# lucidrains/voicebox-pytorch

Hardware: AMD Instinct MI355X
Metric: mel-frames/sec train-step (fwd+bwd+allreduce+clip+Adam) (higher is better)
Workload: dtype f16/bf16 (fp16 forward operands, bf16 backward operands, fp32 accumulate/master); 1 GPU; VoiceBox dim 512 depth 12 heads 16 unconditional, 8x1024 frames per GPU, train; global_batch=8, seq_len=1024, parallelism=dp1

## Files before the change

voicebox-pytorch_amd/csrc/ops.hip:

```cpp
#include "common.hpp"
#include "reduce_roles.hpp"
#include <stdlib.h>

namespace {

VBX_DEV void unpack8_bf16(const uint4 p, float v[8]) {
  const unsigned w[4] = {p.x, p.y, p.z, p.w};
#pragma unroll
  for (int i = 0; i < 4; i++) {
    v[2 * i] = bf16_to_f32((u16)(w[i] & 0xffff));
    v[2 * i + 1] = bf16_to_f32((u16)(w[i] >> 16));
  }
}
VBX_DEV void unpack8_f16(const uint4 p, float v[8]) {
  const unsigned w[4] = {p.x, p.y, p.z, p.w};
#pragma unroll
  for (int i = 0; i < 4; i++) {
    v[2 * i] = f16_to_f32((u16)(w[i] & 0xffff));
    v[2 * i + 1] = f16_to_f32((u16)(w[i] >> 16));
  }
}
VBX_DEV uint4 pack8_h(const float v[8]) {
  return make_uint4(pack_f16x2_sat(v[0], v[1]), pack_f16x2_sat(v[2], v[3]), pack_f16x2_sat(v[4], v[5]), pack_f16x2_sat(v[6], v[7]));
}
// ... 111 lines not shown
  const int lane = threadIdx.x & 63;
  const long r = (long)blockIdx.x * 4 + (threadIdx.x >> 6);
  if (r >= rows) return;
  float s = 0.f;
  for (int d = lane * 4; d < D; d += 256) {
    const float4 a = *reinterpret_cast<const float4*>(x + r * D + d), b = *reinterpret_cast<const float4*>(w + d);
    s += a.x * b.x + a.y * b.y + a.z * b.z + a.w * b.w;
  }
  s = wave_sum(s);
  if (lane == 0) out[r] = s + (bias ? bias[0] : 0.f);
}
__global__ void cond_emb_bwd_kernel(const u16* __restrict__ demb, int ld, const long* __restrict__ ids, int T,
                                    const uint8_t* __restrict__ drop, long null_id, float* __restrict__ gtable, int B, int N, int E) {
  const long total = (long)B * N * E;
  for (long i = blockIdx.x * (long)blockDim.x + threadIdx.x; i < total; i += (long)gridDim.x * blockDim.x) {
    const long row = i / E;
    const int e = (int)(i - row * E);
    const int b = (int)(row / N), n = (int)(row - (long)b * N);
    const bool dropped = drop && drop[b];
    int i0, i1;
    float lam;
    interp_src(n, N, T, i0, i1, lam);
    const float g = bf16_to_f32(demb[row * ld + e]);
    const long id0 = dropped ? null_id : ids[(long)b * T + i0], id1 = dropped ? null_id : ids[(long)b * T + i1];
    if (T == N) {
      atomicAdd(gtable + id0 * E + e, g);
    } else {
      atomicAdd(gtable + id0 * E + e, (1.0f - lam) * g);
      atomicAdd(gtable + id1 * E + e, lam * g);
    }
  }
}

constexpr int CT = 64;
template <int MODE, int KS>
__global__ __launch_bounds__(256) void convpos_fwd_kernel(const float* __restrict__ e, const float* __restrict__ w,
                                                          const float* __restrict__ bias, const uint8_t* __restrict__ mask,
                                                          const float* __restrict__ dxs, float* __restrict__ out, int N,
                                                          int R, int D) {
  extern __shared__ float tile[];
  constexpr int ks = KS;
  const int half = ks / 2;
  const int n0 = blockIdx.x * CT, dbase = blockIdx.y * 64, b = blockIdx.z;
  const int dl = threadIdx.x & 63, ng = threadIdx.x >> 6;
  const int d = dbase + dl;
  const int rows = CT + ks - 1;
  for (int r = ng; r < rows; r += 4) {
    const int n = n0 + r - half;
    float v = 0.f;
    if (n >= 0 && n < N && d < D && (!mask || mask[(long)b * N + n])) v = e[((long)b * N + n) * D + d];
    tile[r * 64 + dl] = v;
  }
  __syncthreads();
  if (d >= D) return;
  float wr[KS];
#pragma unroll
  for (int k = 0; k < ks; k++) wr[k] = w[(long)d * ks + k];
  const float bb = bias[d];
  const int Np = N + R;
  for (int i = 0; i < 16; i++) {
    const int nl = ng * 16 + i, n = n0 + nl;
    if (n >= N) break;
    float acc = bb;
#pragma unroll
    for (int k = 0; k < ks; k++) acc += wr[k] * tile[(nl + k) * 64 + dl];
    const bool m = !mask || mask[(long)b * N + n];
    if (MODE == 0 || MODE == 2) {
      const float ev = e[((long)b * N + n) * D + d];
      out[((long)b * Np + R + n) * D + d] = ev + (m ? (MODE == 2 ? gelu_erf_libm(acc) : gelu_erf(acc)) : 0.f);
    } else {
      const float g = dxs[((long)b * Np + R + n) * D + d];
      out[((long)b * N + n) * D + d] = m ? g * gelu_erf_grad(acc) : 0.f;
    }
  }
}

__global__ void stack_rows_kernel(const float* __restrict__ src, float* __restrict__ dst, int B, int N, int R, int D, int to_stack) {
  const long total = (long)B * N * D / 4;
  const int D4 = D / 4;
  for (long i = blockIdx.x * (long)blockDim.x + threadIdx.x; i < total; i += (long)gridDim.x * blockDim.x) {
    const long row = i / D4;
    const int c = (int)(i - row * D4);
    const int b = (int)(row / N), n = (int)(row - (long)b * N);
    const long wide = ((long)b * (N + R) + R + n) * D4 + c, narrow = i;
    if (to_stack) reinterpret_cast<float4*>(dst)[wide] = reinterpret_cast<const float4*>(src)[narrow];
    else reinterpret_cast<float4*>(dst)[narrow] = reinterpret_cast<const float4*>(src)[wide];
  }
}

__global__ void unet_cat_kernel(const float* __restrict__ x, const float* __restrict__ skip, float scale, u16* __restrict__ o16,
                                u16* __restrict__ ob, long rows, int D) {
  const int cpr = D / 4;
  const long total = rows * 2 * cpr;
  for (long i = blockIdx.x * (long)blockDim.x + threadIdx.x; i < total; i += (long)gridDim.x * blockDim.x) {
    const long row = i / (2 * cpr);
    const int c = (int)(i - row * 2 * cpr);
    const bool second = c >= cpr;
    const int d = (second ? c - cpr : c) * 4;
    float4 v = *reinterpret_cast<const float4*>((second ? skip : x) + row * D + d);
    if (second) { v.x *= scale; v.y *= scale; v.z *= scale; v.w *= scale; }
    const long oo = row * 2 * D + (second ? D : 0) + d;
    if (o16) *reinterpret_cast<uint2*>(o16 + oo) = make_uint2(pack_f16x2_sat(v.x, v.y), pack_f16x2_sat(v.z, v.w));
    if (ob) *reinterpret_cast<uint2*>(ob + oo) = make_uint2(pack_bf16x2(v.x, v.y), pack_bf16x2(v.z, v.w));
  }
}
__global__ void unet_split_kernel(const float* __restrict__ dcat, float scale, float* __restrict__ dx, u16* __restrict__ dxb,
// ... 2 lines not shown
  const long total = rows * cpr;
  for (long i = blockIdx.x * (long)blockDim.x + threadIdx.x; i < total; i += (long)gridDim.x * blockDim.x) {
    const long row = i / cpr;
    const int d = (int)(i - row * cpr) * 4;
    const float4 a = *reinterpret_cast<const float4*>(dcat + row * 2 * D + d);
    float4 b = *reinterpret_cast<const float4*>(dcat + row * 2 * D + D + d);
    b.x *= scale; b.y *= scale; b.z *= scale; b.w *= scale;
    *reinterpret_cast<float4*>(dx + row * D + d) = a;
    if (dxb) *reinterpret_cast<uint2*>(dxb + row * D + d) = make_uint2(pack_bf16x2(a.x, a.y), pack_bf16x2(a.z, a.w));
    *reinterpret_cast<float4*>(dskip + row * D + d) = b;
  }
}
__global__ void unet_addskip_kernel(float* __restrict__ dx, u16* __restrict__ dxb, const float* __restrict__ dskip, long n4) {
  for (long i = blockIdx.x * (long)blockDim.x + threadIdx.x; i < n4; i += (long)gridDim.x * blockDim.x) {
    float4 a = reinterpret_cast<float4*>(dx)[i];
    const float4 b = reinterpret_cast<const float4*>(dskip)[i];
    a.x += b.x; a.y += b.y; a.z += b.z; a.w += b.w;
    reinterpret_cast<float4*>(dx)[i] = a;
    if (dxb) reinterpret_cast<uint2*>(dxb)[i] = make_uint2(pack_bf16x2(a.x, a.y), pack_bf16x2(a.z, a.w));
  }
}

__global__ void regs_fill_kernel(const float* __restrict__ reg, float* __restrict__ xs, int B, int Np, int R, int D) {
  const long total = (long)B * R * D;
  for (long i = blockIdx.x * (long)blockDim.x + threadIdx.x; i < total; i += (long)gridDim.x * blockDim.x) {
    const int b = (int)(i / ((long)R * D));
    const long rd = i - (long)b * R * D;
    xs[(long)b * Np * D + rd] = reg[rd];
  }
}

template <int KS>
__global__ __launch_bounds__(256) void convpos_bwd_kernel(const float* __restrict__ e, const float* __restrict__ w,
                                                          const uint8_t* __restrict__ mask, const float* __restrict__ dxs,
                                                          const float* __restrict__ dpre, float* __restrict__ de,
                                                          u16* __restrict__ deb, float* __restrict__ wpart, int N, int R,
                                                          int D) {
  extern __shared__ float sm[];
  constexpr int ks = KS;
  static_assert(KS <= 31, "wacc holds the taps in [0, KS) and the bias gradient in [31]");
  const int half = ks / 2;
  const int rows = CT + ks - 1;
  float* te = sm;
  float* tp = sm + rows * 64;
  const int n0 = blockIdx.x * CT, dbase = blockIdx.y * 64, b = blockIdx.z;
  const int dl = threadIdx.x & 63, ng = threadIdx.x >> 6;
  const int d = dbase + dl;
  for (int r = ng; r < rows; r += 4) {
    const int n = n0 + r - half;
    float ve = 0.f, vp = 0.f;
    if (n >= 0 && n < N && d < D) {
      if (!mask || mask[(long)b * N + n]) ve = e[((long)b * N + n) * D + d];
      vp = dpre[((long)b * N + n) * D + d];
    }
    te[r * 64 + dl] = ve;
    tp[r * 64 + dl] = vp;
  }
  __syncthreads();
  float wr[KS], wacc[32];
#pragma unroll
  for (int k = 0; k < 32; k++) wacc[k] = 0.f;
  if (d < D) {
#pragma unroll
    for (int k = 0; k < ks; k++) wr[k] = w[(long)d * ks + k];
    const int Np = N + R;
    for (int i = 0; i < 16; i++) {
      const int nl = ng * 16 + i, n = n0 + nl;
      if (n >= N) break;
      float acc = 0.f;
#pragma unroll
      for (int k = 0; k < ks; k++) acc += wr[k] * tp[(nl + 2 * half - k) * 64 + dl];
      const bool m = !mask || mask[(long)b * N + n];
      const float o = dxs[((long)b * Np + R + n) * D + d] + (m ? acc : 0.f);
      de[((long)b * N + n) * D + d] = o;
      if (deb) deb[((long)b * N + n) * D + d] = f32_to_bf16(o);
      const float dp = tp[(nl + half) * 64 + dl];
#pragma unroll
      for (int k = 0; k < ks; k++) wacc[k] += dp * te[(nl + k) * 64 + dl];
      wacc[31] += dp;
    }
  }
  __syncthreads();
  float* red = sm;
#pragma unroll
  for (int k = 0; k < 32; k++) red[(ng * 64 + dl) * 33 + k] = wacc[k];
  __syncthreads();
  const long chunk = (long)b * gridDim.x + blockIdx.x;
  for (int idx = threadIdx.x; idx < 64 * 32; idx += 256) {
    const int c = idx >> 5, k = idx & 31;
    if (dbase + c < D) {
      const float s = red[(0 * 64 + c) * 33 + k] + red[(1 * 64 + c) * 33 + k] + red[(2 * 64 + c) * 33 + k] +
                      red[(3 * 64 + c) * 33 + k];
      wpart[(chunk * D + dbase + c) * 64 + (k == 31 ? 63 : k)] = s;
    }
  }
}

__global__ void conv_wgrad_finalize_kernel(const float* __restrict__ wpart, int chunks, int D, int ks, float* __restrict__ dw,
                                           float* __restrict__ db) {
  const int idx = blockIdx.x * blockDim.x + threadIdx.x;
  if (idx >= D * 64) return;
  const int d = idx >> 6, k = idx & 63;
  if (k >= ks && k != 63) return;
  float s = 0.f;
  int c = 0;
  for (; c + 4 <= chunks; c += 4) {
    float v[4];
#pragma unroll
    for (int u = 0; u < 4; u++) v[u] = wpart[((long)(c + u) * D + d) * 64 + k];
#pragma unroll
    for (int u = 0; u < 4; u++) s += v[u];
  }
  for (; c < chunks; c++) s += wpart[((long)c * D + d) * 64 + k];
  if (k == 63) db[d] = s;
  else dw[(long)d * ks + k] = s;
}

__global__ void dreg_kernel(const float* __restrict__ dxs, float* __restrict__ dreg, int B, int Np, int R, int D) {
  const int i = blockIdx.x * blockDim.x + threadIdx.x;
  if (i >= R * D) return;
  float s = 0.f;
  for (int b = 0; b < B; b++) s += dxs[(long)b * Np * D + i];
  dreg[i] = s;
}

__global__ void time_four_kernel(const float* __restrict__ times, const float* __restrict__ wsin, float* __restrict__ four,
                                 int B, int D) {
  const int i = blockIdx.x * blockDim.x + threadIdx.x;
  if (i >= B * D) return;
  const int b = i / D, j = i - b * D, hd = D / 2;
  const int jj = j < hd ? j : j - hd;
  float f = times[b] * wsin[jj];
  f = f * 2.0f;
  f = f * 3.14159265358979323846f;
  four[i] = j < hd ? sinf(f) : cosf(f);
}
__global__ __launch_bounds__(256) void time_linear_kernel(const float* __restrict__ four, const float* __restrict__ w1,
                                                           const float* __restrict__ b1, float* __restrict__ pre,
                                                           float* __restrict__ temb, int B, int D, int Th) {
  const int lane = threadIdx.x & 63;
  const long o = (long)blockIdx.x * 4 + (threadIdx.x >> 6);
  if (o >= (long)B * Th) return;
  const int b = (int)(o / Th), i = (int)(o - (long)b * Th);
  float s = 0.f;
  for (int j = lane; j < D; j += 64) s += four[(long)b * D + j] * w1[(long)i * D + j];
  s = wave_sum(s);
  if (lane == 0) {
// ... 1118 lines not shown
  VBX_LAUNCH_CHECK();
  return 0;
}

extern "C" int vbx_rowdot(const float* x, const float* w, const float* bias, float* out, long rows, int D, void* stream) {
  VBX_REQUIRE(x && w && out && rows > 0 && D > 0 && D % 4 == 0, "vbx_rowdot: bad args");
  hipLaunchKernelGGL(rowdot_kernel, dim3((unsigned)cdiv(rows, 4L)), dim3(256), 0, ST, x, w, bias, out, rows, D);
  VBX_LAUNCH_CHECK();
  return 0;
}

extern "C" int vbx_cond_emb_bwd(const void* demb_bf16, int ld, const long* ids, int T, const uint8_t* drop_mask, long null_id,
                                float* gtable, int B, int N, int E, void* stream) {
  VBX_REQUIRE(demb_bf16 && ids && gtable && T > 0 && E > 0 && ld >= E, "vbx_cond_emb_bwd: bad args");
  hipLaunchKernelGGL(cond_emb_bwd_kernel, dim3(grid_for((long)B * N * E)), dim3(256), 0, ST, (const u16*)demb_bf16, ld, ids, T,
                     drop_mask, null_id, gtable, B, N, E);
  VBX_LAUNCH_CHECK();
  return 0;
}

#define VBX_CONV_KS_SWITCH(ks, CALL)                                                                                      \
  switch (ks) {                                                                                                           \
    case 1: CALL(1); break;   case 3: CALL(3); break;   case 5: CALL(5); break;   case 7: CALL(7); break;                 \
    case 9: CALL(9); break;   case 11: CALL(11); break; case 13: CALL(13); break; case 15: CALL(15); break;               \
    case 17: CALL(17); break; case 19: CALL(19); break; case 21: CALL(21); break; case 23: CALL(23); break;               \
    case 25: CALL(25); break; case 27: CALL(27); break; case 29: CALL(29); break; default: CALL(31); break;               \
  }
static inline bool conv_ks_ok(int ks) { return ks >= 1 && ks <= 31 && (ks & 1); }

static int convpos_fwd_impl(const float* e, const float* w, const float* bias, const uint8_t* mask, const float* reg, float* xs, int B,
                            int N, int R, int D, int ksize, bool libm, void* stream) {
  VBX_REQUIRE(e && w && bias && xs, "vbx_convpos_fwd: null pointer");
  VBX_REQUIRE(conv_ks_ok(ksize), "vbx_convpos_fwd: conv_pos_embed_kernel_size must be odd and <= 31 (got %d)", ksize);
  VBX_REQUIRE(R == 0 || reg, "vbx_convpos_fwd: register tokens missing");
  dim3 grid(cdiv(N, CT), cdiv(D, 64), B);
#define VBX_CALL(KS)                                                                                                           \
  if (libm)                                                                                                                    \
    hipLaunchKernelGGL((convpos_fwd_kernel<2, KS>), grid, dim3(256), (CT + KS - 1) * 64 * sizeof(float), ST, e, w, bias, mask, \
                       (const float*)nullptr, xs, N, R, D);                                                                    \
  else                                                                                                                         \
    hipLaunchKernelGGL((convpos_fwd_kernel<0, KS>), grid, dim3(256), (CT + KS - 1) * 64 * sizeof(float), ST, e, w, bias, mask, \
                       (const float*)nullptr, xs, N, R, D)
  VBX_CONV_KS_SWITCH(ksize, VBX_CALL)
#undef VBX_CALL
  VBX_LAUNCH_CHECK();
  if (R > 0) {
    hipLaunchKernelGGL(regs_fill_kernel, dim3(grid_for((long)B * R * D)), dim3(256), 0, ST, reg, xs, B, N + R, R, D);
    VBX_LAUNCH_CHECK();
  }
  return 0;
}

extern "C" int vbx_convpos_fwd(const float* e, const float* w, const float* bias, const uint8_t* mask, const float* reg,
                               float* xs, int B, int N, int R, int D, int ksize, void* stream) {
  return convpos_fwd_impl(e, w, bias, mask, reg, xs, B, N, R, D, ksize, false, stream);
}
extern "C" int vbx_convpos_fwd_libm(const float* e, const float* w, const float* bias, const uint8_t* mask, const float* reg,
                                    float* xs, int B, int N, int R, int D, int ksize, void* stream) {
  return convpos_fwd_impl(e, w, bias, mask, reg, xs, B, N, R, D, ksize, true, stream);
}

extern "C" int vbx_stack_input(const float* x, const float* reg, float* xs, int B, int N, int R, int D, void* stream) {
  VBX_REQUIRE(x && xs && B > 0 && N > 0 && R >= 0 && D % 4 == 0 && (R == 0 || reg), "vbx_stack_input: bad args");
  hipLaunchKernelGGL(stack_rows_kernel, dim3(grid_for((long)B * N * D / 4)), dim3(256), 0, ST, x, xs, B, N, R, D, 1);
  VBX_LAUNCH_CHECK();
  if (R > 0) {
    hipLaunchKernelGGL(regs_fill_kernel, dim3(grid_for((long)B * R * D)), dim3(256), 0, ST, reg, xs, B, N + R, R, D);
    VBX_LAUNCH_CHECK();
  }
  return 0;
}

extern "C" int vbx_unet_cat(const float* x, const float* skip, float scale, void* cat_f16, void* cat_bf16, long rows, int D, void* stream) {
  VBX_REQUIRE(x && skip && (cat_f16 || cat_bf16) && rows > 0 && D > 0 && D % 4 == 0, "vbx_unet_cat: bad args");
  hipLaunchKernelGGL(unet_cat_kernel, dim3(grid_for(rows * D / 2)), dim3(256), 0, ST, x, skip, scale, (u16*)cat_f16, (u16*)cat_bf16, rows, D);
  VBX_LAUNCH_CHECK();
  return 0;
}
extern "C" int vbx_unet_split(const float* dcat, float scale, float* dx, void* dx_bf16, float* dskip, long rows, int D, void* stream) {
  VBX_REQUIRE(dcat && dx && dskip && rows > 0 && D > 0 && D % 4 == 0, "vbx_unet_split: bad args");
  hipLaunchKernelGGL(unet_split_kernel, dim3(grid_for(rows * D / 4)), dim3(256), 0, ST, dcat, scale, dx, (u16*)dx_bf16, dskip, rows, D);
  VBX_LAUNCH_CHECK();
  return 0;
}
extern "C" int vbx_unet_addskip(float* dx, void* dx_bf16, const float* dskip, long n, void* stream) {
  VBX_REQUIRE(dx && dskip && n > 0 && n % 4 == 0, "vbx_unet_addskip: bad args");
  hipLaunchKernelGGL(unet_addskip_kernel, dim3(grid_for(n / 4)), dim3(256), 0, ST, dx, (u16*)dx_bf16, dskip, n / 4);
  VBX_LAUNCH_CHECK();
  return 0;
}

extern "C" int vbx_stack_input_bwd(const float* dxs, float* dx, float* dreg, int B, int N, int R, int D, void* stream) {
  VBX_REQUIRE(dxs && dx && B > 0 && N > 0 && R >= 0 && D % 4 == 0, "vbx_stack_input_bwd: bad args");
  hipLaunchKernelGGL(stack_rows_kernel, dim3(grid_for((long)B * N * D / 4)), dim3(256), 0, ST, dxs, dx, B, N, R, D, 0);
  VBX_LAUNCH_CHECK();
  if (R > 0 && dreg) {
    hipLaunchKernelGGL(dreg_kernel, dim3(cdiv((long)R * D, 256)), dim3(256), 0, ST, dxs, dreg, B, N + R, R, D);
    VBX_LAUNCH_CHECK();
  }
  return 0;
}

extern "C" int vbx_convpos_bwd_chunks(int B, int N) { return B * cdiv(N, CT); }

extern "C" int vbx_convpos_bwd(const float* e, const float* w, const float* bias, const uint8_t* mask, const float* dxs,
                               float* dpre_tmp, float* de, void* de_bf16, float* wpart, float* dreg, int B, int N, int R,
                               int D, int ksize, void* stream) {
  VBX_REQUIRE(e && w && bias && dxs && dpre_tmp && de && wpart, "vbx_convpos_bwd: null pointer");
  VBX_REQUIRE(conv_ks_ok(ksize), "vbx_convpos_bwd: conv_pos_embed_kernel_size must be odd and <= 31 (got %d)", ksize);
  dim3 grid(cdiv(N, CT), cdiv(D, 64), B);
  const int rows = CT + ksize - 1;
#define VBX_CALL(KS)                                                                                                            \
  hipLaunchKernelGGL((convpos_fwd_kernel<1, KS>), grid, dim3(256), rows * 64 * sizeof(float), ST, e, w, bias, mask, dxs, dpre_tmp, \
                     N, R, D)
  VBX_CONV_KS_SWITCH(ksize, VBX_CALL)
#undef VBX_CALL
  VBX_LAUNCH_CHECK();
  size_t lds = (size_t)(2 * rows * 64) * sizeof(float);
  if (lds < (size_t)4 * 64 * 33 * sizeof(float)) lds = (size_t)4 * 64 * 33 * sizeof(float);
  static bool attr[32] = {};
#define VBX_CALL(KS)                                                                                                              \
  {                                                                                                                               \
    if (!attr[KS]) {                                                                                                              \
      (void)hipFuncSetAttribute(reinterpret_cast<const void*>(convpos_bwd_kernel<KS>), hipFuncAttributeMaxDynamicSharedMemorySize, \
                                (int)lds);                                                                                        \
      attr[KS] = true;                                                                                                            \
    }                                                                                                                             \
    hipLaunchKernelGGL(convpos_bwd_kernel<KS>, grid, dim3(256), lds, ST, e, w, mask, dxs, dpre_tmp, de, (u16*)de_bf16, wpart, N,   \
                       R, D);                                                                                                     \
  }
  VBX_CONV_KS_SWITCH(ksize, VBX_CALL)
#undef VBX_CALL
  VBX_LAUNCH_CHECK();
  if (R > 0 && dreg) {
    hipLaunchKernelGGL(dreg_kernel, dim3(cdiv((long)R * D, 256)), dim3(256), 0, ST, dxs, dreg, B, N + R, R, D);
    VBX_LAUNCH_CHECK();
  }
  return 0;
}

extern "C" int vbx_conv_wgrad_finalize(const float* wpart, int chunks, int D, int ksize, float* dw, float* db, void* stream) {
  VBX_REQUIRE(wpart && dw && db && ksize < 63, "vbx_conv_wgrad_finalize: bad args");
  hipLaunchKernelGGL(conv_wgrad_finalize_kernel, dim3(cdiv((long)D * 64, 256)), dim3(256), 0, ST, wpart, chunks, D, ksize, dw, db);
  VBX_LAUNCH_CHECK();
  return 0;
}

extern "C" int vbx_time_embed_fwd(const float* times, const float* w_sin, const float* w1, const float* b1, float* four,
                                  float* pre, float* temb, int B, int D, int Th, void* stream) {
  VBX_REQUIRE(times && w_sin && w1 && b1 && four && pre && temb && D % 2 == 0, "vbx_time_embed_fwd: bad args");
  hipLaunchKernelGGL(time_four_kernel, dim3(cdiv((long)B * D, 256)), dim3(256), 0, ST, times, w_sin, four, B, D);
  VBX_LAUNCH_CHECK();
  hipLaunchKernelGGL(time_linear_kernel, dim3(cdiv((long)B * Th, 4)), dim3(256), 0, ST, four, w1, b1, pre, temb, B, D, Th);
  VBX_LAUNCH_CHECK();
  return 0;
}

extern "C" int vbx_time_embed_bwd_scratch_floats(int B, int D) { return (1 + TB_SLICES) * B * D; }

extern "C" int vbx_time_embed_bwd(const float* times, const float* w_sin, const float* w1, const float* four,
                                  const float* pre, const float* dtemb, float* dw_sin, float* dw1, float* db1,
                                  float* scratch, int B, int D, int Th, void* stream) {
  VBX_REQUIRE(times && w_sin && w1 && four && pre && dtemb && dw_sin && dw1 && db1 && scratch, "vbx_time_embed_bwd: null");
  hipLaunchKernelGGL(time_bwd_w1_kernel, dim3(cdiv((long)Th * D, 256)), dim3(256), 0, ST, four, pre, dtemb, dw1, db1, B, D, Th);
  VBX_LAUNCH_CHECK();
  hipLaunchKernelGGL(time_bwd_four_kernel, dim3(cdiv(D, 64), B, TB_SLICES), dim3(64), 0, ST, w1, pre, dtemb, scratch + (long)B * D,
                     B, D, Th);
  VBX_LAUNCH_CHECK();
  hipLaunchKernelGGL(sum_rows_kernel, dim3(cdiv((long)B * D, 64)), dim3(256), 0, ST, scratch + (long)B * D, (long)TB_SLICES,
                     (long)B * D, scratch, (long)B * D, 0);
  VBX_LAUNCH_CHECK();
  hipLaunchKernelGGL(time_bwd_wsin_kernel, dim3(cdiv(D / 2, 256)), dim3(256), 0, ST, times, four, scratch, dw_sin, B, D);
  VBX_LAUNCH_CHECK();
  return 0;
}

// ... 434 lines not shown
```

voicebox-pytorch_amd/csrc/runtime.hip:

```cpp
#include "common.hpp"
#include <stdlib.h>
#include <algorithm>
#include <string.h>
#include <string>
#include <vector>

namespace {

inline size_t al256(size_t x) { return (x + 255) & ~(size_t)255; }

struct Carver {
  char* base;
  size_t off = 0;
  explicit Carver(void* b) : base((char*)b) {}
  template <class T>
  T* take(size_t n) {
    off = al256(off);
    T* p = base ? (T*)(base + off) : nullptr;
    off += n * sizeof(T);
    return p;
  }
};

struct Dims {
// ... 44 lines not shown
    w.layer[l].w1 = c.take<u16>((size_t)2 * d.Fp * d.D);
    w.layer[l].w1h = c.take<u16>((size_t)2 * d.Fp * d.D);
    w.layer[l].b1 = c.take<float>(2 * d.Fp);
    w.layer[l].w2 = c.take<u16>((size_t)d.D * d.Fp);
    w.layer[l].w2h = c.take<u16>((size_t)d.D * d.Fp);
    w.layer[l].glw = m->gateloop ? c.take<u16>((size_t)3 * d.D * d.D) : nullptr;
    w.layer[l].glwh = m->gateloop ? c.take<u16>((size_t)3 * d.D * d.D) : nullptr;
    if (m->unet && l >= d.L / 2) {
      w.layer[l].skw = c.take<u16>((size_t)2 * d.D * d.D);
      w.layer[l].skwh = c.take<u16>((size_t)2 * d.D * d.D);
    }
  }
  w.bytes = al256(c.off);
}

struct ALayer {
  u16 *hn1, *hn1h, *q16, *k16, *qb, *kb, *v, *vh, *o, *oh, *hn2, *hn2h, *h1, *g, *gh;
  float *qrn, *krn, *lse;
  unsigned *dbr = nullptr, *dbc = nullptr;
  u16 *hg = nullptr, *hgh = nullptr;
  float *glp = nullptr, *glh = nullptr, *gls = nullptr;
};
struct Acts {
  u16 *embed_in, *embed_inh;
  u16 *xcb = nullptr, *dxc = nullptr;
  float *e, *four, *pre, *temb, *ada;
  std::vector<float*> xs;
  std::vector<float*> xc, dskip;
  u16 *cat16 = nullptr, *catb = nullptr;
  float* dcat = nullptr;
  std::vector<ALayer> layer;
  u16 *hf, *hfh;
  float *pred, *per_b;
  float *dx, *dq, *dk, *delta, *slabs, *npart, *npart2, *cpart, *dada, *dtemb, *cs_scratch, *cs_layers, *gpart, *tmp2d, *ada_scratch, *dpre, *de, *wpart,
      *tscratch;
  u16 *dxb, *dg, *dh1, *dhn, *dO, *dqkv, *deb, *dpb, *gl_dp, *demb;
  char* attn_scratch = nullptr;
  u16* dxb2 = nullptr;
  float* gl_ds;
  size_t slab_floats;
  size_t np_stride = 0, cp_stride = 0, cs_stride = 0, gp_stride = 0;
  size_t bytes;
};

int wgrad_splits(long I, long J, long K) {
  const long tiles = ((I + 127) / 128) * ((J + 127) / 128);
  const long smax = (K + 511) / 512;
  int best = 1;
  double best_cost = 1e30;
  for (int s = 1; s <= 16 && s <= smax; s++) {
    const long W = tiles * s;
    const long n = (W + 255) / 256;
    const double eff = n >= 3 ? 1.0 : (n == 2 ? 0.85 : 0.6);
    const double ksteps = (double)((K + s - 1) / s) / 32.0;
    const double gemm = (double)n * ksteps * 0.27 / eff;
    const double slab = (double)s * (double)I * (double)J * 8.0 / 4.0e6;
    const double cost = gemm + slab;
    if (cost < best_cost) { best_cost = cost; best = s; }
  }
  return best;
}

bool group_wgrad() { return vbx_gemm_path() != 1; }
struct WgradGroup {
  vbx_gemm_desc d[4];
  int n = 0;
};
// ... 93 lines not shown
    auto upd = [&](long I, long J, long K) {
      const int s1 = wgrad_splits(I, J, K);
      const size_t n = (size_t)(s1 > s3 ? s1 : s3) * I * J;
      if (n > sf) sf = n;
    };
    upd(3 * d.I, d.D, d.M); upd(d.D, d.I, d.M); upd(2 * d.Fp, d.D, d.M); upd(d.D, d.Fp, d.M);
    upd(d.D, d.Ke, d.M0); upd(d.Dop, d.D, d.M0);
    if (d.Lc) upd(d.D, d.Kp, 2 * d.M0);
    if (m->gateloop) upd(3 * d.D, d.D, d.M);
    if (m->unet) upd(d.D, 2 * d.D, d.M);
    a.slab_floats = sf;
    a.slabs = c.take<float>(4 * sf);
    const size_t nreg = (m->gateloop || m->unet) ? 1 : (size_t)d.L;
    a.np_stride = (size_t)d.B * vbx_rmsnorm_bwd_chunks(d.Np) * 2 * d.D;
    a.cp_stride = (size_t)d.B * vbx_rmsnorm_bwd_chunks(d.Np) * d.D;
    a.npart = c.take<float>(a.np_stride * nreg);
    a.npart2 = c.take<float>(a.np_stride * nreg);
    a.cpart = c.take<float>(a.cp_stride * nreg);
    a.dada = c.take<float>((size_t)d.B * d.J);
    a.dtemb = c.take<float>((size_t)d.B * d.Th);
    size_t cs = (size_t)vbx_colsum_scratch_floats((int)d.M, 2 * d.Fp);
    if (cs < (size_t)vbx_geglu_bwd_colsum_slabs() * 2 * d.Fp) cs = (size_t)vbx_geglu_bwd_colsum_slabs() * 2 * d.Fp;
    a.cs_scratch = c.take<float>(cs);
    a.cs_stride = (size_t)vbx_geglu_bwd_colsum_slabs() * 2 * d.Fp;
    a.cs_layers = c.take<float>(a.cs_stride * nreg);
    {
      const int r1 = vbx_qknorm_rope_bwd_gpart_rows(d.B), r2 = d.B * vbx_attn_bwd_fused_tiles(d.Np);
      a.gp_stride = (size_t)2 * (r1 > r2 ? r1 : r2) * d.H * 64;
      a.gpart = c.take<float>(a.gp_stride * nreg);
    }
    a.tmp2d = c.take<float>(2 * d.D);
    a.ada_scratch = c.take<float>(std::max((size_t)vbx_adaln_proj_bwd_scratch_floats(d.B, d.Th, 4 * d.D),
                                           (size_t)vbx_adaln_dtemb_all_scratch_floats(d.L, d.B, d.Th, 4 * d.D)));
    a.dpre = c.take<float>((size_t)d.M0 * d.D);
    a.de = c.take<float>((size_t)d.M0 * d.D);
    a.deb = c.take<u16>((size_t)d.M0 * d.D);
    a.dpb = c.take<u16>((size_t)d.M0 * d.Dop);
    a.wpart = c.take<float>((size_t)vbx_convpos_bwd_chunks(d.B, d.N) * d.D * 64);
    a.tscratch = c.take<float>((size_t)vbx_time_embed_bwd_scratch_floats(d.B, d.D));
    a.gl_ds = m->gateloop ? c.take<float>((size_t)d.M * d.D) : nullptr;
    a.gl_dp = m->gateloop ? c.take<u16>((size_t)d.M * 3 * d.D) : nullptr;
    a.demb = d.E ? c.take<u16>((size_t)d.M0 * d.E) : nullptr;
    if (d.Lc) {
      a.xcb = c.take<u16>((size_t)2 * d.M0 * d.Kp);
      a.dxc = c.take<u16>((size_t)2 * d.M0 * d.D);
    }
    a.dxb2 = c.take<u16>((size_t)d.M * d.D);
    a.attn_scratch = c.take<char>(vbx_attn_bwd_scratch_bytes(d.B, d.H, d.Np));
    if (m->unet) {
      a.catb = c.take<u16>((size_t)d.M * 2 * d.D);
      a.dcat = c.take<float>((size_t)d.M * 2 * d.D);
      for (int p = 0; p < d.L / 2; p++) a.dskip[p] = c.take<float>((size_t)d.M * d.D);
    }
  }
  a.bytes = al256(c.off);
}

struct ProfRec {
  const char* label;
  hipEvent_t e0, e1;
};
struct Prof {
  bool on = false;
  std::vector<ProfRec> recs;
};
Prof g_prof;
struct ProfScope {
// ... 521 lines not shown
    if (l == 0) {
      ProfScope ps("adaLN dtemb (all)", st);
      CK(vbx_adaln_dtemb_all(w.adah, a.dada, a.dtemb, a.ada_scratch, d.L, d.B, d.Th, 4 * d.D, stream));
    }
    return 0;
  }
  return vbx_adaln_proj_bwd(m->stack_only ? io->cond : a.temb, w.adah + (size_t)l * 4 * d.D * d.Th, dada_l,
                            m->adaln_factors ? nullptr : Gd + o[VBX_L_G1W], Gd + o[VBX_L_G1B], a.dtemb,
                            a.ada_scratch, d.B, d.Th, 4 * d.D, l == d.L - 1 ? 0 : 1, stream);
}

extern "C" int vbx_model_backward_embed(const vbx_model* m, const vbx_io* io, void* stream) {
  CK(check_model(m));
  VBX_REQUIRE(m->training && m->grads && io && (m->stack_only ? io->dx != nullptr : io->times != nullptr),
              "vbx_model_backward_embed: needs a training forward");
  hipStream_t st = (hipStream_t)stream;
  const Dims d = dims_of(m);
  WPack w;
  carve_wpack(m, w);
  Acts a;
  carve_acts(m, a);
  const float* P = m->params;
  float* Gd = m->grads;
  const long* G = m->off;
  if (m->stack_only) {
    CK(vbx_stack_input_bwd(a.dx, io->dx, d.R ? Gd + G[VBX_P_REG] : nullptr, d.B, d.N, d.R, d.D, stream));
    if (!m->plain_norm && io->dcond &&
        hipMemcpyAsync(io->dcond, a.dtemb, (size_t)d.B * d.Th * sizeof(float), hipMemcpyDeviceToDevice, st) != hipSuccess) {
      vbx_set_error("vbx_model_backward_embed: copy of d(cond) failed");
      return VBX_EINVAL;
    }
    return 0;
  }
  CK(vbx_convpos_bwd(a.e, P + G[VBX_P_CONVW], P + G[VBX_P_CONVB], io->attn_mask, a.dx, a.dpre, a.de, a.deb, a.wpart,
                     d.R ? Gd + G[VBX_P_REG] : nullptr, d.B, d.N, d.R, d.D, d.ks, stream));
  CK(vbx_conv_wgrad_finalize(a.wpart, vbx_convpos_bwd_chunks(d.B, d.N), d.D, d.ks, Gd + G[VBX_P_CONVW], Gd + G[VBX_P_CONVB], stream));
  CK(wgrad(a.deb, d.D, a.embed_in, d.Ke, d.D, d.Ke, d.M0, a.slabs, Gd + G[VBX_P_EMBW], d.D, d.Ke, 0, 0, st));
  if (d.E) {
    WPack w;
    carve_wpack(m, w);
    CK(gemm_nn_bf16(a.deb, d.D, w.embb + d.Din, d.Ke, (int)d.M0, d.E, d.D, a.demb, d.E, st));
    if (hipMemsetAsync(Gd + G[VBX_P_CEMB], 0, (size_t)m->V1 * d.E * sizeof(float), st) != hipSuccess) {
      vbx_set_error("vbx_model_backward_embed: memset of the embedding gradient failed");
      return VBX_EINVAL;
    }
    CK(vbx_cond_emb_bwd(a.demb, d.E, io->cond_ids, io->T, io->drop_mask, io->null_id, Gd + G[VBX_P_CEMB], d.B, d.N, d.E, stream));
  }
  if (d.Lc) {
    WPack w;
    carve_wpack(m, w);
    CK(gemm_nn_bf16(a.deb, d.D, w.embb, d.Ke, (int)d.M0, d.D, d.D, a.dxc, d.D, st));
    CK(gemm_nn_bf16(a.deb, d.D, w.embb + d.D + d.E, d.Ke, (int)d.M0, d.D, d.D, a.dxc + (size_t)d.M0 * d.D, d.D, st));
    vbx_gemm_desc g{};
    g.mode = VBX_GEMM_TN; g.epilogue = VBX_EPI_SPLITK; g.M = d.D; g.N = d.Kp; g.K = (int)(2 * d.M0); g.lda = d.D; g.ldb = d.Kp;
    g.A = a.dxc; g.B = a.xcb; g.C = a.slabs; g.splits = wgrad_splits(d.D, d.Kp, 2 * d.M0);
    CK(vbx_gemm(&g, st));
    CK(vbx_proj_in_wgrad_reduce(a.slabs, g.splits, d.D, d.Lc, Gd + G[VBX_P_PINW], Gd + G[VBX_P_PINB], stream));
  }
  CK(vbx_colsum_f32(a.de, (int)d.M0, d.D, d.D, Gd + G[VBX_P_EMBB], a.cs_scratch, stream));
  CK(vbx_time_embed_bwd(io->times, P + G[VBX_P_SINW], P + G[VBX_P_T1W], a.four, a.pre, a.dtemb, Gd + G[VBX_P_SINW],
                        Gd + G[VBX_P_T1W], Gd + G[VBX_P_T1B], a.tscratch, d.B, d.D, d.Th, stream));
  return 0;
}

extern "C" int vbx_model_adam_segments(const vbx_model* m, long n_flat, vbx_adam_seg* out, int max_segs, long* total_blocks) {
  CK(check_model(m));
  VBX_REQUIRE(n_flat > 0 && total_blocks, "vbx_model_adam_segments: bad args");
// ... 118 lines not shown
```

Baseline: 961,300 mel-frames/s.

## Fuse conv-pos backward pre-activation recompute into one kernel with register-tiled frames

The backward pass for the positional depthwise conv now recomputes the pre-activation inside the main backward kernel, using a halo tile of the input. This removes the separate MODE-1 forward launch and the fp32 dpre buffer round-trip through global memory. Both forward and backward are re-tiled: each thread owns two channels and eight frames, with float4 tile fills and float2 LDS accesses, and weight-grad partials are pre-reduced with warp shuffles into a 32-wide wpart layout. The cost is redundant conv compute over the halo rows, more registers per thread, and a new requirement that D be a multiple of 4.

After: 970,100 mel-frames/s (median of 6 runs). Within noise of the previous version (+0.9%).

```diff
diff --git a/voicebox-pytorch_amd/csrc/ops.hip b/voicebox-pytorch_amd/csrc/ops.hip
--- a/voicebox-pytorch_amd/csrc/ops.hip
+++ b/voicebox-pytorch_amd/csrc/ops.hip
@@ -167,46 +167,85 @@
   }
 }
 
-constexpr int CT = 64;
-template <int MODE, int KS>
+constexpr int CV_RUN = 128, CV_CW = 32, CV_FR = 8, CV_P = 36;
+
+template <int ROWS>
+__device__ __forceinline__ void conv_fill_tile(float* __restrict__ tile, const float* __restrict__ src, const uint8_t* __restrict__ mrow,
+                                               int nfirst, int N, int D, int dbase) {
+  constexpr int IT = (ROWS * 8 + 255) / 256;
+  float4 v[IT];
+  bool ok[IT];
+#pragma unroll
+  for (int it = 0; it < IT; it++) {
+    const int idx = threadIdx.x + it * 256, r = idx >> 3, c4 = idx & 7;
+    const int n = nfirst + r, d = dbase + c4 * 4;
+    const int nc = min(max(n, 0), N - 1), dc = min(d, D - 4);
+    ok[it] = n >= 0 && n < N && d < D && (!mrow || mrow[nc]);
+    v[it] = *reinterpret_cast<const float4*>(src + (long)nc * D + dc);
+  }
+#pragma unroll
+  for (int it = 0; it < IT; it++) {
+    const int idx = threadIdx.x + it * 256, r = idx >> 3, c4 = idx & 7;
+    if (idx < ROWS * 8) *reinterpret_cast<float4*>(tile + r * CV_P + c4 * 4) = ok[it] ? v[it] : make_float4(0.f, 0.f, 0.f, 0.f);
+  }
+}
+
+template <int LIBM, int KS>
 __global__ __launch_bounds__(256) void convpos_fwd_kernel(const float* __restrict__ e, const float* __restrict__ w,
                                                           const float* __restrict__ bias, const uint8_t* __restrict__ mask,
-                                                          const float* __restrict__ dxs, float* __restrict__ out, int N,
-                                                          int R, int D) {
+                                                          float* __restrict__ out, int N, int R, int D) {
   extern __shared__ float tile[];
-  constexpr int ks = KS;
-  const int half = ks / 2;
-  const int n0 = blockIdx.x * CT, dbase = blockIdx.y * 64, b = blockIdx.z;
-  const int dl = threadIdx.x & 63, ng = threadIdx.x >> 6;
-  const int d = dbase + dl;
-  const int rows = CT + ks - 1;
-  for (int r = ng; r < rows; r += 4) {
-    const int n = n0 + r - half;
-    float v = 0.f;
-    if (n >= 0 && n < N && d < D && (!mask || mask[(long)b * N + n])) v = e[((long)b * N + n) * D + d];
-    tile[r * 64 + dl] = v;
-  }
+  constexpr int half = KS / 2, rows = CV_RUN + KS - 1;
+  const int n0 = blockIdx.x * CV_RUN, dbase = blockIdx.y * CV_CW, b = blockIdx.z;
+  const int q = threadIdx.x & 15, f0 = (threadIdx.x >> 4) * CV_FR;
+  const int d = dbase + 2 * q;
+  const uint8_t* mrow = mask ? mask + (long)b * N : nullptr;
+  const float* eb = e + (long)b * N * D;
+  float wr[2][KS], acc[CV_FR][2];
+  if (d < D) {
+#pragma unroll
+    for (int k = 0; k < KS; k++) {
+      wr[0][k] = w[(long)d * KS + k];
+      wr[1][k] = w[(long)(d + 1) * KS + k];
+    }
+#pragma unroll
+    for (int i = 0; i < CV_FR; i++) {
+      acc[i][0] = bias[d];
+      acc[i][1] = bias[d + 1];
+    }
+  }
+  conv_fill_tile<rows>(tile, eb, mrow, n0 - half, N, D, dbase);
   __syncthreads();
   if (d >= D) return;
-  float wr[KS];
-#pragma unroll
-  for (int k = 0; k < ks; k++) wr[k] = w[(long)d * ks + k];
-  const float bb = bias[d];
+#pragma unroll
+  for (int j = 0; j < CV_FR + KS - 1; j++) {
+    const float2 x = *reinterpret_cast<const float2*>(tile + (f0 + j) * CV_P + 2 * q);
+#pragma unroll
+    for (int i = 0; i < CV_FR; i++) {
+      const int k = j - i;
+      if (k >= 0 && k < KS) {
+        acc[i][0] += wr[0][k] * x.x;
+        acc[i][1] += wr[1][k] * x.y;
+      }
+    }
+  }
   const int Np = N + R;
-  for (int i = 0; i < 16; i++) {
-    const int nl = ng * 16 + i, n = n0 + nl;
+#pragma unroll
+  for (int i = 0; i < CV_FR; i++) {
+    const int n = n0 + f0 + i;
     if (n >= N) break;
-    float acc = bb;
-#pragma unroll
-    for (int k = 0; k < ks; k++) acc += wr[k] * tile[(nl + k) * 64 + dl];
-    const bool m = !mask || mask[(long)b * N + n];
-    if (MODE == 0 || MODE == 2) {
-      const float ev = e[((long)b * N + n) * D + d];
-      out[((long)b * Np + R + n) * D + d] = ev + (m ? (MODE == 2 ? gelu_erf_libm(acc) : gelu_erf(acc)) : 0.f);
+    const bool m = !mrow || mrow[n];
+    float2 o;
+    if (m) {
+      const float2 ev = *reinterpret_cast<const float2*>(tile + (f0 + i + half) * CV_P + 2 * q);
+      o.x = ev.x + (LIBM ? gelu_erf_libm(acc[i][0]) : gelu_erf(acc[i][0]));
+      o.y = ev.y + (LIBM ? gelu_erf_libm(acc[i][1]) : gelu_erf(acc[i][1]));
     } else {
-      const float g = dxs[((long)b * Np + R + n) * D + d];
-      out[((long)b * N + n) * D + d] = m ? g * gelu_erf_grad(acc) : 0.f;
-    }
+      const float2 ev = *reinterpret_cast<const float2*>(eb + (long)n * D + d);
+      o.x = ev.x + 0.f;
+      o.y = ev.y + 0.f;
+    }
+    *reinterpret_cast<float2*>(out + ((long)b * Np + R + n) * D + d) = o;
   }
 }
 
@@ -275,66 +314,144 @@
 
 template <int KS>
 __global__ __launch_bounds__(256) void convpos_bwd_kernel(const float* __restrict__ e, const float* __restrict__ w,
-                                                          const uint8_t* __restrict__ mask, const float* __restrict__ dxs,
-                                                          const float* __restrict__ dpre, float* __restrict__ de,
+                                                          const float* __restrict__ bias, const uint8_t* __restrict__ mask,
+                                                          const float* __restrict__ dxs, float* __restrict__ de,
                                                           u16* __restrict__ deb, float* __restrict__ wpart, int N, int R,
                                                           int D) {
   extern __shared__ float sm[];
-  constexpr int ks = KS;
-  static_assert(KS <= 31, "wacc holds the taps in [0, KS) and the bias gradient in [31]");
-  const int half = ks / 2;
-  const int rows = CT + ks - 1;
+  constexpr int half = KS / 2;
+  constexpr int RE = CV_RUN + 4 * half, RP = CV_RUN + 2 * half;
+  constexpr int PB = (RP + 15) / 16;
   float* te = sm;
-  float* tp = sm + rows * 64;
-  const int n0 = blockIdx.x * CT, dbase = blockIdx.y * 64, b = blockIdx.z;
-  const int dl = threadIdx.x & 63, ng = threadIdx.x >> 6;
-  const int d = dbase + dl;
-  for (int r = ng; r < rows; r += 4) {
-    const int n = n0 + r - half;
-    float ve = 0.f, vp = 0.f;
-    if (n >= 0 && n < N && d < D) {
-      if (!mask || mask[(long)b * N + n]) ve = e[((long)b * N + n) * D + d];
-      vp = dpre[((long)b * N + n) * D + d];
-    }
-    te[r * 64 + dl] = ve;
-    tp[r * 64 + dl] = vp;
-  }
+  float* tp = sm + RE * CV_P;
+  const int n0 = blockIdx.x * CV_RUN, dbase = blockIdx.y * CV_CW, b = blockIdx.z;
+  const int q = threadIdx.x & 15, g = threadIdx.x >> 4;
+  const int d = dbase + 2 * q;
+  const bool active = d < D;
+  const int Np = N + R;
+  const uint8_t* mrow = mask ? mask + (long)b * N : nullptr;
+  const float* dxb = dxs + ((long)b * Np + R) * D;
+  float wr[2][KS];
+  float bb[2] = {0.f, 0.f};
+  if (active) {
+#pragma unroll
+    for (int k = 0; k < KS; k++) {
+      wr[0][k] = w[(long)d * KS + k];
+      wr[1][k] = w[(long)(d + 1) * KS + k];
+    }
+    bb[0] = bias[d];
+    bb[1] = bias[d + 1];
+  }
+  conv_fill_tile<RE>(te, e + (long)b * N * D, mrow, n0 - 2 * half, N, D, dbase);
+  conv_fill_tile<RP>(tp, dxb, mrow, n0 - half, N, D, dbase);
   __syncthreads();
-  float wr[KS], wacc[32];
-#pragma unroll
-  for (int k = 0; k < 32; k++) wacc[k] = 0.f;
-  if (d < D) {
-#pragma unroll
-    for (int k = 0; k < ks; k++) wr[k] = w[(long)d * ks + k];
-    const int Np = N + R;
-    for (int i = 0; i < 16; i++) {
-      const int nl = ng * 16 + i, n = n0 + nl;
+  if (active) {
+    const int rb = g * PB;
+    float acc[PB][2];
+#pragma unroll
+    for (int i = 0; i < PB; i++) {
+      acc[i][0] = bb[0];
+      acc[i][1] = bb[1];
+    }
+#pragma unroll
+    for (int j = 0; j < PB + KS - 1; j++) {
+      const float2 x = *reinterpret_cast<const float2*>(te + min(rb + j, RE - 1) * CV_P + 2 * q);
+#pragma unroll
+      for (int i = 0; i < PB; i++) {
+        const int k = j - i;
+        if (k >= 0 && k < KS) {
+          acc[i][0] += wr[0][k] * x.x;
+          acc[i][1] += wr[1][k] * x.y;
+        }
+      }
+    }
+#pragma unroll
+    for (int i = 0; i < PB; i++) {
+      const int r = rb + i;
+      if (r < RP) {
+        float2* pp = reinterpret_cast<float2*>(tp + r * CV_P + 2 * q);
+        const float2 gv = *pp;
+        *pp = make_float2(gv.x * gelu_erf_grad(acc[i][0]), gv.y * gelu_erf_grad(acc[i][1]));
+      }
+    }
+  }
+  __syncthreads();
+  float wacc[2][32];
+#pragma unroll
+  for (int k = 0; k < 32; k++) wacc[0][k] = wacc[1][k] = 0.f;
+  if (active) {
+    const int f0 = g * CV_FR;
+    float acc[CV_FR][2];
+#pragma unroll
+    for (int i = 0; i < CV_FR; i++) acc[i][0] = acc[i][1] = 0.f;
+#pragma unroll
+    for (int j = CV_FR + 2 * half - 1; j >= 0; j--) {
+      const float2 x = *reinterpret_cast<const float2*>(tp + (f0 + j) * CV_P + 2 * q);
+#pragma unroll
+      for (int i = 0; i < CV_FR; i++) {
+        const int k = i + 2 * half - j;
+        if (k >= 0 && k < KS) {
+          acc[i][0] += wr[0][k] * x.x;
+          acc[i][1] += wr[1][k] * x.y;
+        }
+      }
+    }
+    float2 dp[CV_FR];
+#pragma unroll
+    for (int i = 0; i < CV_FR; i++) {
+      dp[i] = *reinterpret_cast<const float2*>(tp + (f0 + i + half) * CV_P + 2 * q);
+      wacc[0][31] += dp[i].x;
+      wacc[1][31] += dp[i].y;
+    }
+#pragma unroll
+    for (int j = 0; j < CV_FR + KS - 1; j++) {
+      const float2 x = *reinterpret_cast<const float2*>(te + (f0 + half + j) * CV_P + 2 * q);
+#pragma unroll
+      for (int i = 0; i < CV_FR; i++) {
+        const int k = j - i;
+        if (k >= 0 && k < KS) {
+          wacc[0][k] += dp[i].x * x.x;
+          wacc[1][k] += dp[i].y * x.y;
+        }
+      }
+    }
+#pragma unroll
+    for (int i = 0; i < CV_FR; i++) {
+      const int n = n0 + f0 + i;
       if (n >= N) break;
-      float acc = 0.f;
-#pragma unroll
-      for (int k = 0; k < ks; k++) acc += wr[k] * tp[(nl + 2 * half - k) * 64 + dl];
-      const bool m = !mask || mask[(long)b * N + n];
-      const float o = dxs[((long)b * Np + R + n) * D + d] + (m ? acc : 0.f);
-      de[((long)b * N + n) * D + d] = o;
-      if (deb) deb[((long)b * N + n) * D + d] = f32_to_bf16(o);
-      const float dp = tp[(nl + half) * 64 + dl];
-#pragma unroll
-      for (int k = 0; k < ks; k++) wacc[k] += dp * te[(nl + k) * 64 + dl];
-      wacc[31] += dp;
-    }
-  }
+      const bool m = !mrow || mrow[n];
+      const float2 gv = *reinterpret_cast<const float2*>(dxb + (long)n * D + d);
+      const float ox = gv.x + (m ? acc[i][0] : 0.f), oy = gv.y + (m ? acc[i][1] : 0.f);
+      *reinterpret_cast<float2*>(de + ((long)b * N + n) * D + d) = make_float2(ox, oy);
+      if (deb) *reinterpret_cast<uint32_t*>(deb + ((long)b * N + n) * D + d) = (uint32_t)f32_to_bf16(ox) | ((uint32_t)f32_to_bf16(oy) << 16);
+    }
+  }
+#pragma unroll
+  for (int c = 0; c < 2; c++)
+#pragma unroll
+    for (int k = 0; k < 32; k++) {
+      if (k >= KS && k != 31) continue;
+      float v = wacc[c][k];
+      v += __shfl_xor(v, 16);
+      v += __shfl_xor(v, 32);
+      wacc[c][k] = v;
+    }
   __syncthreads();
   float* red = sm;
-#pragma unroll
-  for (int k = 0; k < 32; k++) red[(ng * 64 + dl) * 33 + k] = wacc[k];
+  const int wv = threadIdx.x >> 6;
+  if ((threadIdx.x & 63) < 16) {
+#pragma unroll
+    for (int c = 0; c < 2; c++)
+#pragma unroll
+      for (int k = 0; k < 32; k++) red[(wv * 32 + 2 * q + c) * 33 + k] = wacc[c][k];
+  }
   __syncthreads();
   const long chunk = (long)b * gridDim.x + blockIdx.x;
-  for (int idx = threadIdx.x; idx < 64 * 32; idx += 256) {
+  for (int idx = threadIdx.x; idx < 32 * 32; idx += 256) {
     const int c = idx >> 5, k = idx & 31;
     if (dbase + c < D) {
-      const float s = red[(0 * 64 + c) * 33 + k] + red[(1 * 64 + c) * 33 + k] + red[(2 * 64 + c) * 33 + k] +
-                      red[(3 * 64 + c) * 33 + k];
-      wpart[(chunk * D + dbase + c) * 64 + (k == 31 ? 63 : k)] = s;
+      const float s = red[(0 * 32 + c) * 33 + k] + red[(1 * 32 + c) * 33 + k] + red[(2 * 32 + c) * 33 + k] + red[(3 * 32 + c) * 33 + k];
+      wpart[(chunk * D + dbase + c) * 32 + k] = s;
     }
   }
 }
@@ -342,20 +459,22 @@
 __global__ void conv_wgrad_finalize_kernel(const float* __restrict__ wpart, int chunks, int D, int ks, float* __restrict__ dw,
                                            float* __restrict__ db) {
   const int idx = blockIdx.x * blockDim.x + threadIdx.x;
-  if (idx >= D * 64) return;
-  const int d = idx >> 6, k = idx & 63;
-  if (k >= ks && k != 63) return;
+  if (idx >= D * 32) return;
+  const int d = idx >> 5, k = idx & 31;
+  if (k >= ks && k != 31) return;
+  const long stride = (long)D * 32;
+  const float* p = wpart + idx;
   float s = 0.f;
   int c = 0;
-  for (; c + 4 <= chunks; c += 4) {
-    float v[4];
-#pragma unroll
-    for (int u = 0; u < 4; u++) v[u] = wpart[((long)(c + u) * D + d) * 64 + k];
-#pragma unroll
-    for (int u = 0; u < 4; u++) s += v[u];
-  }
-  for (; c < chunks; c++) s += wpart[((long)c * D + d) * 64 + k];
-  if (k == 63) db[d] = s;
+  for (; c + 8 <= chunks; c += 8) {
+    float v[8];
+#pragma unroll
+    for (int u = 0; u < 8; u++) v[u] = p[(c + u) * stride];
+#pragma unroll
+    for (int u = 0; u < 8; u++) s += v[u];
+  }
+  for (; c < chunks; c++) s += p[c * stride];
+  if (k == 31) db[d] = s;
   else dw[(long)d * ks + k] = s;
 }
 
@@ -1540,15 +1659,16 @@
                             int N, int R, int D, int ksize, bool libm, void* stream) {
   VBX_REQUIRE(e && w && bias && xs, "vbx_convpos_fwd: null pointer");
   VBX_REQUIRE(conv_ks_ok(ksize), "vbx_convpos_fwd: conv_pos_embed_kernel_size must be odd and <= 31 (got %d)", ksize);
+  VBX_REQUIRE(B > 0 && N > 0 && D > 0 && D % 4 == 0, "vbx_convpos_fwd: dim must be a multiple of 4 (got %d)", D);
   VBX_REQUIRE(R == 0 || reg, "vbx_convpos_fwd: register tokens missing");
-  dim3 grid(cdiv(N, CT), cdiv(D, 64), B);
-#define VBX_CALL(KS)                                                                                                           \
-  if (libm)                                                                                                                    \
-    hipLaunchKernelGGL((convpos_fwd_kernel<2, KS>), grid, dim3(256), (CT + KS - 1) * 64 * sizeof(float), ST, e, w, bias, mask, \
-                       (const float*)nullptr, xs, N, R, D);                                                                    \
-  else                                                                                                                         \
-    hipLaunchKernelGGL((convpos_fwd_kernel<0, KS>), grid, dim3(256), (CT + KS - 1) * 64 * sizeof(float), ST, e, w, bias, mask, \
-                       (const float*)nullptr, xs, N, R, D)
+  dim3 grid(cdiv(N, CV_RUN), cdiv(D, CV_CW), B);
+#define VBX_CALL(KS)                                                                                                               \
+  if (libm)                                                                                                                        \
+    hipLaunchKernelGGL((convpos_fwd_kernel<1, KS>), grid, dim3(256), (CV_RUN + KS - 1) * CV_P * sizeof(float), ST, e, w, bias, mask, \
+                       xs, N, R, D);                                                                                               \
+  else                                                                                                                             \
+    hipLaunchKernelGGL((convpos_fwd_kernel<0, KS>), grid, dim3(256), (CV_RUN + KS - 1) * CV_P * sizeof(float), ST, e, w, bias, mask, \
+                       xs, N, R, D)
   VBX_CONV_KS_SWITCH(ksize, VBX_CALL)
 #undef VBX_CALL
   VBX_LAUNCH_CHECK();
@@ -1609,23 +1729,18 @@
   return 0;
 }
 
-extern "C" int vbx_convpos_bwd_chunks(int B, int N) { return B * cdiv(N, CT); }
+extern "C" int vbx_convpos_bwd_chunks(int B, int N) { return B * cdiv(N, CV_RUN); }
 
 extern "C" int vbx_convpos_bwd(const float* e, const float* w, const float* bias, const uint8_t* mask, const float* dxs,
                                float* dpre_tmp, float* de, void* de_bf16, float* wpart, float* dreg, int B, int N, int R,
                                int D, int ksize, void* stream) {
-  VBX_REQUIRE(e && w && bias && dxs && dpre_tmp && de && wpart, "vbx_convpos_bwd: null pointer");
+  (void)dpre_tmp;
+  VBX_REQUIRE(e && w && bias && dxs && de && wpart, "vbx_convpos_bwd: null pointer");
   VBX_REQUIRE(conv_ks_ok(ksize), "vbx_convpos_bwd: conv_pos_embed_kernel_size must be odd and <= 31 (got %d)", ksize);
-  dim3 grid(cdiv(N, CT), cdiv(D, 64), B);
-  const int rows = CT + ksize - 1;
-#define VBX_CALL(KS)                                                                                                            \
-  hipLaunchKernelGGL((convpos_fwd_kernel<1, KS>), grid, dim3(256), rows * 64 * sizeof(float), ST, e, w, bias, mask, dxs, dpre_tmp, \
-                     N, R, D)
-  VBX_CONV_KS_SWITCH(ksize, VBX_CALL)
-#undef VBX_CALL
-  VBX_LAUNCH_CHECK();
-  size_t lds = (size_t)(2 * rows * 64) * sizeof(float);
-  if (lds < (size_t)4 * 64 * 33 * sizeof(float)) lds = (size_t)4 * 64 * 33 * sizeof(float);
+  VBX_REQUIRE(B > 0 && N > 0 && D > 0 && D % 4 == 0, "vbx_convpos_bwd: dim must be a multiple of 4 (got %d)", D);
+  dim3 grid(cdiv(N, CV_RUN), cdiv(D, CV_CW), B);
+  size_t lds = (size_t)(2 * CV_RUN + 6 * (ksize / 2)) * CV_P * sizeof(float);
+  if (lds < (size_t)4 * 32 * 33 * sizeof(float)) lds = (size_t)4 * 32 * 33 * sizeof(float);
   static bool attr[32] = {};
 #define VBX_CALL(KS)                                                                                                              \
   {                                                                                                                               \
@@ -1634,8 +1749,7 @@
                                 (int)lds);                                                                                        \
       attr[KS] = true;                                                                                                            \
     }                                                                                                                             \
-    hipLaunchKernelGGL(convpos_bwd_kernel<KS>, grid, dim3(256), lds, ST, e, w, mask, dxs, dpre_tmp, de, (u16*)de_bf16, wpart, N,   \
-                       R, D);                                                                                                     \
+    hipLaunchKernelGGL(convpos_bwd_kernel<KS>, grid, dim3(256), lds, ST, e, w, bias, mask, dxs, de, (u16*)de_bf16, wpart, N, R, D); \
   }
   VBX_CONV_KS_SWITCH(ksize, VBX_CALL)
 #undef VBX_CALL
@@ -1648,8 +1762,8 @@
 }
 
 extern "C" int vbx_conv_wgrad_finalize(const float* wpart, int chunks, int D, int ksize, float* dw, float* db, void* stream) {
-  VBX_REQUIRE(wpart && dw && db && ksize < 63, "vbx_conv_wgrad_finalize: bad args");
-  hipLaunchKernelGGL(conv_wgrad_finalize_kernel, dim3(cdiv((long)D * 64, 256)), dim3(256), 0, ST, wpart, chunks, D, ksize, dw, db);
+  VBX_REQUIRE(wpart && dw && db && ksize <= 31, "vbx_conv_wgrad_finalize: bad args");
+  hipLaunchKernelGGL(conv_wgrad_finalize_kernel, dim3(cdiv((long)D * 32, 256)), dim3(256), 0, ST, wpart, chunks, D, ksize, dw, db);
   VBX_LAUNCH_CHECK();
   return 0;
 }
diff --git a/voicebox-pytorch_amd/csrc/runtime.hip b/voicebox-pytorch_amd/csrc/runtime.hip
--- a/voicebox-pytorch_amd/csrc/runtime.hip
+++ b/voicebox-pytorch_amd/csrc/runtime.hip
@@ -100,7 +100,7 @@
   std::vector<ALayer> layer;
   u16 *hf, *hfh;
   float *pred, *per_b;
-  float *dx, *dq, *dk, *delta, *slabs, *npart, *npart2, *cpart, *dada, *dtemb, *cs_scratch, *cs_layers, *gpart, *tmp2d, *ada_scratch, *dpre, *de, *wpart,
+  float *dx, *dq, *dk, *delta, *slabs, *npart, *npart2, *cpart, *dada, *dtemb, *cs_scratch, *cs_layers, *gpart, *tmp2d, *ada_scratch, *de, *wpart,
       *tscratch;
   u16 *dxb, *dg, *dh1, *dhn, *dO, *dqkv, *deb, *dpb, *gl_dp, *demb;
   char* attn_scratch = nullptr;
@@ -260,7 +260,6 @@
     a.tmp2d = c.take<float>(2 * d.D);
     a.ada_scratch = c.take<float>(std::max((size_t)vbx_adaln_proj_bwd_scratch_floats(d.B, d.Th, 4 * d.D),
                                            (size_t)vbx_adaln_dtemb_all_scratch_floats(d.L, d.B, d.Th, 4 * d.D)));
-    a.dpre = c.take<float>((size_t)d.M0 * d.D);
     a.de = c.take<float>((size_t)d.M0 * d.D);
     a.deb = c.take<u16>((size_t)d.M0 * d.D);
     a.dpb = c.take<u16>((size_t)d.M0 * d.Dop);
@@ -848,7 +847,7 @@
     }
     return 0;
   }
-  CK(vbx_convpos_bwd(a.e, P + G[VBX_P_CONVW], P + G[VBX_P_CONVB], io->attn_mask, a.dx, a.dpre, a.de, a.deb, a.wpart,
+  CK(vbx_convpos_bwd(a.e, P + G[VBX_P_CONVW], P + G[VBX_P_CONVB], io->attn_mask, a.dx, nullptr, a.de, a.deb, a.wpart,
                      d.R ? Gd + G[VBX_P_REG] : nullptr, d.B, d.N, d.R, d.D, d.ks, stream));
   CK(vbx_conv_wgrad_finalize(a.wpart, vbx_convpos_bwd_chunks(d.B, d.N), d.D, d.ks, Gd + G[VBX_P_CONVW], Gd + G[VBX_P_CONVB], stream));
   CK(wgrad(a.deb, d.D, a.embed_in, d.Ke, d.D, d.Ke, d.M0, a.slabs, Gd + G[VBX_P_EMBW], d.D, d.Ke, 0, 0, st));
```
